# Robinatp/YOLO_Tensorflow

Hardware: AMD Instinct MI355X
Metric: images_per_sec (higher is better)
Workload: dtype bf16; 1 GPU; YOLOv3 416x416 batch=32 per GPU, bf16: conv stack + head decode + threshold + TF-NMS; global_batch=32, input=uint8 NHWC resident in HBM, weights=seeded synthetic darknet stream (seed 0), parallelism=dp1

## Files before the change

### yolo_tensorflow_amd/csrc/conv_block.hip

```cpp
#include "kernels.h"
#include "device_common.h"
#include <type_traits>

constexpr int CB_B = 13;
constexpr int CB_T = CB_B + 2;
constexpr int CB_TPIX = CB_T * CB_T;
constexpr int CB_TSUB = (CB_TPIX + 15) / 16;
constexpr int CB_OPIX = CB_B * CB_B;
constexpr int CB_OSUB = (CB_OPIX + 15) / 16;
constexpr int CB_C = 128, CB_M = 64;
constexpr int CB_NW = 8;
constexpr int CB_NJ = 6;
constexpr int CB_X_BYTES = CB_TSUB * 16 * CB_C * 2;
constexpr int CB_MPITCH = CB_M * 2 + 16;
constexpr int CB_MID_BYTES = CB_TSUB * 16 * CB_MPITCH;
constexpr int CB_W1PITCH = CB_C * 2 + 16;
constexpr int CB_W1_BYTES = CB_M * CB_W1PITCH;
constexpr int CB_OPITCH = CB_C * 2 + 16;
constexpr int CB_OUT_BYTES = CB_OSUB * 16 * CB_OPITCH;
constexpr int CB_B1_BYTES = CB_M * 4, CB_B2_BYTES = CB_C * 4;
constexpr int CB_LDS = CB_X_BYTES + CB_MID_BYTES + CB_W1_BYTES + CB_B1_BYTES + CB_B2_BYTES + CB_OUT_BYTES;

template <bool H16>
__global__ __launch_bounds__(64 * CB_NW) void conv_resblock_c128(const BlockArgs a)
{
#if defined(__HIP_DEVICE_COMPILE__)
    extern __shared__ __attribute__((aligned(16))) char smem[];
    if constexpr (H16) fp16_saturating_mode();
    const int tid = threadIdx.x, lane = tid & 63, wave = __builtin_amdgcn_readfirstlane(tid >> 6);
    const int l15 = lane & 15, lq = lane >> 4;
    const int wc = wave & 3, wp = wave >> 2;
    char *const lx_ = smem, *const lmid_ = lx_ + CB_X_BYTES, *const lw1_ = lmid_ + CB_MID_BYTES, *const lb1_ = lw1_ + CB_W1_BYTES, *const lb2_ = lb1_ + CB_B1_BYTES, *const lout_ = lb2_ + CB_B2_BYTES;
    const float slope1 = act_slope(a.act1), slope2 = act_slope(a.act2);
    const int bx = (a.W + CB_B - 1) / CB_B, by = (a.H + CB_B - 1) / CB_B, per_img = bx * by, nblocks = a.N * per_img;
    const int nt = (nblocks - (int)blockIdx.x + (int)gridDim.x - 1) / (int)gridDim.x;

    for (int g = tid; g < CB_M * 16; g += 64 * CB_NW) {
        const int row = g >> 4, piece = g & 15;
        *(uint4 *)(lw1_ + row * CB_W1PITCH + piece * 16) = *(const uint4 *)((const bf16_t *)a.w1 + (size_t)row * a.Kpad1 + piece * 8);
    }
    bf16x8 fw2[2][18];
#pragma unroll
    for (int ct = 0; ct < 2; ++ct)
#pragma unroll
        for (int ks = 0; ks < 18; ++ks)
            fw2[ct][ks] = *(const bf16x8 *)((const bf16_t *)a.w2 + (size_t)(wc * 32 + ct * 16 + l15) * a.Kpad2 + ks * 32 + lq * 8);
    if (tid < CB_M) *(float *)(lb1_ + tid * 4) = a.b1[tid];
    if (tid < CB_C) *(float *)(lb2_ + tid * 4) = a.b2[tid];

    __amdgpu_buffer_rsrc_t rx = buf_rsrc(a.x);
    __amdgpu_buffer_rsrc_t ro = buf_rsrc(a.out);

    struct Blk { int n, y0, x0; };
    auto blk_of = [&](int j) { const int b = (int)blockIdx.x + j * (int)gridDim.x; Blk q; q.n = b / per_img; const int r = b - q.n * per_img; q.y0 = (r / bx) * CB_B; q.x0 = (r - (r / bx) * bx) * CB_B; return q; };
    auto fetch_x = [&](const Blk &q, lds_char *dst) {
        const int cl = lane >> 4, chunk = lane & 15;
#pragma unroll 1
        for (int id = wave; id < CB_T * 4; id += CB_NW) {
            const int r = id >> 2, c = (id & 3) * 4 + cl;
            const int iy = q.y0 - 1 + r, ix = q.x0 - 1 + c;
            const bool ok = (unsigned)iy < (unsigned)a.H && (unsigned)ix < (unsigned)a.W;
            const unsigned off = ok ? (unsigned)((((q.n * a.H + iy) * a.W + ix) * a.x_stride + ((chunk ^ ((c - r) & 7)) * 8)) * 2) : 0x80000000u;
            if (c < CB_T) __builtin_amdgcn_raw_ptr_buffer_load_lds(rx, (lds_void *)(dst + (r * CB_T + (id & 3) * 4) * 256), 16, off, 0, 0, 0);
        }
    };

    typedef const __attribute__((address_space(3))) bf16x8 *lds_frag_p;
    uint32_t mida[CB_NJ];
#pragma unroll
    for (int j = 0; j < CB_NJ; ++j) {
        int q = (wp * CB_NJ + j) * 16 + l15; if (q >= CB_OPIX) q = CB_OPIX - 1;
        const int oy = (q * 5042) >> 16, ox = q - oy * CB_B;
        mida[j] = (uint32_t)(uintptr_t)(lds_char *)lmid_ + (uint32_t)((oy * CB_T + ox) * CB_MPITCH + lq * 16);
        asm volatile("" : "+v"(mida[j]));
    }

    auto block = [&](int it, const lds_char *__restrict__ lx, lds_char *__restrict__ lx_dma, lds_char *__restrict__ lmid, const lds_char *__restrict__ mid_rd,
                     const lds_char *__restrict__ lw1, const lds_char *__restrict__ lb1, const lds_char *__restrict__ lb2, lds_char *__restrict__ lout) {
        const Blk q = blk_of(it);
        static_assert((CB_OPIX * 16 + 64 * CB_NW - 1) / (64 * CB_NW) == 6, "vmcnt below counts the stores of one thread");
        if (it > 0) __builtin_amdgcn_s_waitcnt(waitcnt_imm(6, 0));
        __builtin_amdgcn_s_barrier();
        {
            const int u = wave;
            f32x4 acc[2][4];
#pragma unroll
            for (int s = 0; s < 2; ++s)
#pragma unroll
                for (int ct = 0; ct < 4; ++ct) acc[s][ct] = f32x4{0.f, 0.f, 0.f, 0.f};
            int p0 = (2 * u) * 16 + l15;
            asm volatile("" : "+v"(p0));
            const int p1 = p0 + 16;
            bf16x8 xf[2][2], wf[2][4];
            auto frags = [&](int kk) {
                xf[kk & 1][0] = *(lds_frag_p)(lx + p0 * 256 + (((kk * 4 + lq) ^ (p0 & 7)) << 4));
                xf[kk & 1][1] = *(lds_frag_p)(lx + p1 * 256 + (((kk * 4 + lq) ^ (p1 & 7)) << 4));
#pragma unroll
                for (int ct = 0; ct < 4; ++ct) wf[kk & 1][ct] = *(lds_frag_p)(lw1 + (ct * 16 + l15) * CB_W1PITCH + (kk * 4 + lq) * 16);
            };
            frags(0);
            __builtin_amdgcn_sched_barrier(0);
#pragma unroll
            for (int kk = 0; kk < 4; ++kk) {
                if (kk + 1 < 4) frags(kk + 1);
#pragma unroll
                for (int ct = 0; ct < 4; ++ct) {
                    acc[0][ct] = mma16<H16>(wf[kk & 1][ct], xf[kk & 1][0], acc[0][ct]);
                    acc[1][ct] = mma16<H16>(wf[kk & 1][ct], xf[kk & 1][1], acc[1][ct]);
                }
                __builtin_amdgcn_sched_barrier(0);
            }
#pragma unroll
            for (int s = 0; s < 2; ++s) {
                const int p = s ? p1 : p0;
                if (2 * u + s >= CB_TSUB) continue;
                const int r = (p * 4370) >> 16, col = p - r * CB_T;
                const bool inside = p < CB_TPIX && (unsigned)(q.y0 - 1 + r) < (unsigned)a.H && (unsigned)(q.x0 - 1 + col) < (unsigned)a.W;
#pragma unroll
                for (int ct = 0; ct < 4; ++ct) {
                    uint2 pk = leaky_pack4<H16>(acc[s][ct], *(const __attribute__((address_space(3))) f32x4 *)(lb1 + (ct * 16 + lq * 4) * 4), slope1);
                    if (!inside) pk = uint2{0u, 0u};
                    *(__attribute__((address_space(3))) uint2 *)(lmid + p * CB_MPITCH + (ct * 16 + lq * 4) * 2) = pk;
                }
            }
        }
        __builtin_amdgcn_s_waitcnt(waitcnt_imm(63, 0));
        __builtin_amdgcn_s_barrier();
        if (it + 1 < nt) fetch_x(blk_of(it + 1), lx_dma);
        f32x4 acc2[2][CB_NJ];
#pragma unroll
        for (int ct = 0; ct < 2; ++ct)
#pragma unroll
            for (int j = 0; j < CB_NJ; ++j) acc2[ct][j] = f32x4{0.f, 0.f, 0.f, 0.f};
        bf16x8 fg[3][2];
        auto koff = [](int ks) { const int t = ks >> 1, h = ks & 1, kh = t / 3, kw = t - kh * 3; return (kh * CB_T + kw) * CB_MPITCH + h * 64; };
#pragma unroll
        for (int j = 0; j < 2; ++j) fg[0][j] = *(lds_frag_p)(mid_rd + mida[j] + koff(0));
        __builtin_amdgcn_sched_barrier(0);
#pragma unroll
        for (int ks = 0; ks < 18; ++ks)
#pragma unroll
            for (int g = 0; g < 3; ++g) {
                const int gn = (g + 1) % 3, ksn = g == 2 ? ks + 1 : ks;
                if (ksn < 18) {
#pragma unroll
                    for (int j = 0; j < 2; ++j) fg[gn][j] = *(lds_frag_p)(mid_rd + mida[gn * 2 + j] + koff(ksn));
                }
#pragma unroll
                for (int j = 0; j < 2; ++j) { acc2[0][g * 2 + j] = mma16<H16>(fw2[0][ks], fg[g][j], acc2[0][g * 2 + j]); acc2[1][g * 2 + j] = mma16<H16>(fw2[1][ks], fg[g][j], acc2[1][g * 2 + j]); }
                __builtin_amdgcn_sched_barrier(0);
            }
        auto stage_out = [&](int ct) {
            const f32x4 bv = *(const __attribute__((address_space(3))) f32x4 *)(lb2 + (wc * 32 + ct * 16 + lq * 4) * 4);
#pragma unroll
            for (int j = 0; j < CB_NJ; ++j)
                if (wp * CB_NJ + j < CB_OSUB)
                    *(__attribute__((address_space(3))) uint2 *)(lout + ((wp * CB_NJ + j) * 16 + l15) * CB_OPITCH + (wc * 32 + ct * 16 + lq * 4) * 2) = leaky_pack4<H16>(acc2[ct][j], bv, slope2);
        };
        stage_out(0);
        constexpr int NPIECE = (CB_OPIX * 16 + 64 * CB_NW - 1) / (64 * CB_NW);
        u32x4_t rsv[NPIECE];
#pragma unroll
        for (int k = 0; k < NPIECE; ++k) {
            int g = tid + k * 64 * CB_NW;
            asm volatile("" : "+v"(g));
            const int px = g >> 4, piece = g & 15;
            const int oy = (px * 5042) >> 16, ox = px - oy * CB_B;
            const unsigned pix = (unsigned)((q.n * a.H + q.y0 + oy) * a.W + q.x0 + ox);
            rsv[k] = __builtin_amdgcn_raw_buffer_load_b128(rx, (px < CB_OPIX && q.y0 + oy < a.H && q.x0 + ox < a.W) ? (pix * a.x_stride + piece * 8) * 2 : 0x80000000u, 0, 0);
        }
        stage_out(1);
        __builtin_amdgcn_s_waitcnt(waitcnt_imm(63, 0));
        __builtin_amdgcn_s_barrier();
#pragma unroll
        for (int k = 0; k < NPIECE; ++k) {
            int g = tid + k * 64 * CB_NW;
            asm volatile("" : "+v"(g));
            const int px = g >> 4, piece = g & 15;
            const int oy = (px * 5042) >> 16, ox = px - oy * CB_B;
            const bool ok = px < CB_OPIX && q.y0 + oy < a.H && q.x0 + ox < a.W;
            const unsigned pix = (unsigned)((q.n * a.H + q.y0 + oy) * a.W + q.x0 + ox);
            const u32x4_t r = rsv[k];
            u32x4_t o = *(const __attribute__((address_space(3))) u32x4_t *)(lout + (px < CB_OPIX ? px : 0) * CB_OPITCH + piece * 16);
#pragma unroll
            for (int e = 0; e < 4; ++e) o[e] = pack16x2<H16>(unpack16_lo<H16>(o[e]) + unpack16_lo<H16>(r[e]), unpack16_hi<H16>(o[e]) + unpack16_hi<H16>(r[e]));
            __builtin_amdgcn_raw_buffer_store_b128(o, ro, ok ? (pix * a.out_stride + piece * 8) * 2 : 0x80000000u, 0, OUT_STORE_AUX);
        }
    };
    if (nt > 0) fetch_x(blk_of(0), (lds_char *)lx_);
    __builtin_amdgcn_s_waitcnt(waitcnt_imm(0, 0));
    for (int it = 0; it < nt; ++it) block(it, (const lds_char *)lx_, (lds_char *)lx_, (lds_char *)lmid_, (const lds_char *)(uintptr_t)0, (const lds_char *)lw1_, (const lds_char *)lb1_, (const lds_char *)lb2_, (lds_char *)lout_);
#endif
}

bool conv_resblock_ok(const BlockArgs &a)
{
    const double px = (double)a.N * a.H * a.W;
    if (px * a.x_stride * 2.0 >= 2147483648.0 || px * a.out_stride * 2.0 >= 2147483648.0) return false;
    const long cover = (long)((a.H + CB_B - 1) / CB_B) * ((a.W + CB_B - 1) / CB_B) * CB_B * CB_B;
    if (a.H <= 0 || a.W <= 0 || cover * 100 > (long)a.H * a.W * 115) return false;
    return (a.dt == DT_BF16 || a.dt == DT_F16) && a.C == CB_C && a.Cmid == CB_M &&
           a.Kpad1 >= CB_C && a.Kpad2 >= 9 * CB_M && (a.x_stride % 8) == 0 && a.x_stride >= CB_C && (a.out_stride % 8) == 0 && a.out_stride >= CB_C;
}

hipError_t launch_conv_resblock(const BlockArgs &a, hipStream_t s)
{
    if (!conv_resblock_ok(a)) return hipErrorInvalidValue;
    const bool h16 = a.dt == DT_F16;
    const void *k = h16 ? (const void *)conv_resblock_c128<true> : (const void *)conv_resblock_c128<false>;
    { hipError_t e = conv_opt_in_lds(k, CB_LDS); if (e != hipSuccess) return e; }
    long blocks = (long)a.N * ((a.H + CB_B - 1) / CB_B) * ((a.W + CB_B - 1) / CB_B);
    if (blocks > 256) blocks = 256;
    if (h16) hipLaunchKernelGGL(conv_resblock_c128<true>, dim3((unsigned)blocks), dim3(64 * CB_NW), CB_LDS, s, a);
    else hipLaunchKernelGGL(conv_resblock_c128<false>, dim3((unsigned)blocks), dim3(64 * CB_NW), CB_LDS, s, a);
    return hipGetLastError();
}
```

Baseline: 12560 img/s.

## Add four-wave half-height resblock form to fit two workgroups per CU

Templates the fused 1x1+3x3 residual block kernel on a wave-group count, adding a four-wave variant that processes a 6x13 output strip. In that variant the mid and output LDS buffers are aliased, behind an extra barrier, so two workgroups fit on one CU. At launch, an occupancy query picks the four-wave form with a grid of twice the CU count whenever two blocks can be resident, and falls back to the eight-wave form otherwise. The aim is latency hiding across workgroups. The cost is more halo rows per output pixel, an extra barrier, and the register pressure that comes with launch_bounds(…,2).

```diff
diff --git a/yolo_tensorflow_amd/csrc/conv_block.hip b/yolo_tensorflow_amd/csrc/conv_block.hip
--- a/yolo_tensorflow_amd/csrc/conv_block.hip
+++ b/yolo_tensorflow_amd/csrc/conv_block.hip
@@ -1,38 +1,54 @@
 #include "kernels.h"
 #include "device_common.h"
 #include <type_traits>
+#include <map>
+#include <mutex>
 
 constexpr int CB_B = 13;
 constexpr int CB_T = CB_B + 2;
-constexpr int CB_TPIX = CB_T * CB_T;
-constexpr int CB_TSUB = (CB_TPIX + 15) / 16;
-constexpr int CB_OPIX = CB_B * CB_B;
-constexpr int CB_OSUB = (CB_OPIX + 15) / 16;
 constexpr int CB_C = 128, CB_M = 64;
-constexpr int CB_NW = 8;
-constexpr int CB_NJ = 6;
-constexpr int CB_X_BYTES = CB_TSUB * 16 * CB_C * 2;
 constexpr int CB_MPITCH = CB_M * 2 + 16;
-constexpr int CB_MID_BYTES = CB_TSUB * 16 * CB_MPITCH;
 constexpr int CB_W1PITCH = CB_C * 2 + 16;
 constexpr int CB_W1_BYTES = CB_M * CB_W1PITCH;
 constexpr int CB_OPITCH = CB_C * 2 + 16;
-constexpr int CB_OUT_BYTES = CB_OSUB * 16 * CB_OPITCH;
 constexpr int CB_B1_BYTES = CB_M * 4, CB_B2_BYTES = CB_C * 4;
-constexpr int CB_LDS = CB_X_BYTES + CB_MID_BYTES + CB_W1_BYTES + CB_B1_BYTES + CB_B2_BYTES + CB_OUT_BYTES;
-
-template <bool H16>
-__global__ __launch_bounds__(64 * CB_NW) void conv_resblock_c128(const BlockArgs a)
+template <int NP> struct CbGeom {
+    static constexpr int BR = NP == 2 ? CB_B : 6;
+    static constexpr int TR = BR + 2;
+    static constexpr int TPIX = TR * CB_T;
+    static constexpr int TSUB = (TPIX + 15) / 16;
+    static constexpr int OPIX = BR * CB_B;
+    static constexpr int OSUB = (OPIX + 15) / 16;
+    static constexpr int NW = 4 * NP;
+    static constexpr int NJ = (OSUB + NP - 1) / NP;
+    static constexpr int NG = (NJ + 1) / 2;
+    static constexpr int NPIECE = (OPIX * 16 + 64 * NW - 1) / (64 * NW);
+    static constexpr int X_BYTES = TSUB * 16 * CB_C * 2;
+    static constexpr int MID_BYTES = TSUB * 16 * CB_MPITCH;
+    static constexpr int OUT_BYTES = OSUB * 16 * CB_OPITCH;
+    static constexpr bool ALIAS = NP == 1;
+    static constexpr int MIDOUT_BYTES = ALIAS ? (MID_BYTES > OUT_BYTES ? MID_BYTES : OUT_BYTES) : MID_BYTES + OUT_BYTES;
+    static constexpr int LDS = X_BYTES + MIDOUT_BYTES + CB_W1_BYTES + CB_B1_BYTES + CB_B2_BYTES;
+    static_assert(2 * NW >= TSUB, "stage 1: wave u takes halo sub-tiles 2u, 2u + 1");
+    static_assert(TPIX <= 240 && OPIX < 176, "the divisions by 15 and 13 below are multiplications");
+};
+static_assert(CbGeom<2>::LDS == 162048 && CbGeom<2>::LDS <= 160 * 1024, "eight-wave form: one workgroup per CU");
+static_assert(CbGeom<1>::LDS == 72704 && 2 * CbGeom<1>::LDS <= 160 * 1024, "four-wave form: two workgroups per CU");
+
+template <bool H16, int NP>
+__global__ __launch_bounds__(64 * CbGeom<NP>::NW, 2) void conv_resblock_c128(const BlockArgs a)
 {
 #if defined(__HIP_DEVICE_COMPILE__)
+    typedef CbGeom<NP> G;
+    constexpr int CB_NW = G::NW, CB_NJ = G::NJ, CB_TSUB = G::TSUB, CB_TPIX = G::TPIX, CB_OPIX = G::OPIX, CB_OSUB = G::OSUB, CB_TR = G::TR, CB_BR = G::BR, NPIECE = G::NPIECE;
     extern __shared__ __attribute__((aligned(16))) char smem[];
     if constexpr (H16) fp16_saturating_mode();
     const int tid = threadIdx.x, lane = tid & 63, wave = __builtin_amdgcn_readfirstlane(tid >> 6);
     const int l15 = lane & 15, lq = lane >> 4;
     const int wc = wave & 3, wp = wave >> 2;
-    char *const lx_ = smem, *const lmid_ = lx_ + CB_X_BYTES, *const lw1_ = lmid_ + CB_MID_BYTES, *const lb1_ = lw1_ + CB_W1_BYTES, *const lb2_ = lb1_ + CB_B1_BYTES, *const lout_ = lb2_ + CB_B2_BYTES;
+    char *const lx_ = smem, *const lmid_ = lx_ + G::X_BYTES, *const lout_ = G::ALIAS ? lmid_ : lmid_ + G::MID_BYTES, *const lw1_ = lmid_ + G::MIDOUT_BYTES, *const lb1_ = lw1_ + CB_W1_BYTES, *const lb2_ = lb1_ + CB_B1_BYTES;
     const float slope1 = act_slope(a.act1), slope2 = act_slope(a.act2);
-    const int bx = (a.W + CB_B - 1) / CB_B, by = (a.H + CB_B - 1) / CB_B, per_img = bx * by, nblocks = a.N * per_img;
+    const int bx = (a.W + CB_B - 1) / CB_B, by = (a.H + CB_BR - 1) / CB_BR, per_img = bx * by, nblocks = a.N * per_img;
     const int nt = (nblocks - (int)blockIdx.x + (int)gridDim.x - 1) / (int)gridDim.x;
 
     for (int g = tid; g < CB_M * 16; g += 64 * CB_NW) {
@@ -52,11 +68,11 @@
     __amdgpu_buffer_rsrc_t ro = buf_rsrc(a.out);
 
     struct Blk { int n, y0, x0; };
-    auto blk_of = [&](int j) { const int b = (int)blockIdx.x + j * (int)gridDim.x; Blk q; q.n = b / per_img; const int r = b - q.n * per_img; q.y0 = (r / bx) * CB_B; q.x0 = (r - (r / bx) * bx) * CB_B; return q; };
+    auto blk_of = [&](int j) { const int b = (int)blockIdx.x + j * (int)gridDim.x; Blk q; q.n = b / per_img; const int r = b - q.n * per_img; q.y0 = (r / bx) * CB_BR; q.x0 = (r - (r / bx) * bx) * CB_B; return q; };
     auto fetch_x = [&](const Blk &q, lds_char *dst) {
         const int cl = lane >> 4, chunk = lane & 15;
 #pragma unroll 1
-        for (int id = wave; id < CB_T * 4; id += CB_NW) {
+        for (int id = wave; id < CB_TR * 4; id += CB_NW) {
             const int r = id >> 2, c = (id & 3) * 4 + cl;
             const int iy = q.y0 - 1 + r, ix = q.x0 - 1 + c;
             const bool ok = (unsigned)iy < (unsigned)a.H && (unsigned)ix < (unsigned)a.W;
@@ -78,8 +94,7 @@
     auto block = [&](int it, const lds_char *__restrict__ lx, lds_char *__restrict__ lx_dma, lds_char *__restrict__ lmid, const lds_char *__restrict__ mid_rd,
                      const lds_char *__restrict__ lw1, const lds_char *__restrict__ lb1, const lds_char *__restrict__ lb2, lds_char *__restrict__ lout) {
         const Blk q = blk_of(it);
-        static_assert((CB_OPIX * 16 + 64 * CB_NW - 1) / (64 * CB_NW) == 6, "vmcnt below counts the stores of one thread");
-        if (it > 0) __builtin_amdgcn_s_waitcnt(waitcnt_imm(6, 0));
+        if (it > 0) __builtin_amdgcn_s_waitcnt(waitcnt_imm(NPIECE, 0));
         __builtin_amdgcn_s_barrier();
         {
             const int u = wave;
@@ -132,22 +147,23 @@
         for (int ct = 0; ct < 2; ++ct)
 #pragma unroll
             for (int j = 0; j < CB_NJ; ++j) acc2[ct][j] = f32x4{0.f, 0.f, 0.f, 0.f};
-        bf16x8 fg[3][2];
+        bf16x8 fg[G::NG][2];
         auto koff = [](int ks) { const int t = ks >> 1, h = ks & 1, kh = t / 3, kw = t - kh * 3; return (kh * CB_T + kw) * CB_MPITCH + h * 64; };
 #pragma unroll
         for (int j = 0; j < 2; ++j) fg[0][j] = *(lds_frag_p)(mid_rd + mida[j] + koff(0));
+        auto in_group = [](int g, int j) { return g * 2 + j < CB_NJ; };
         __builtin_amdgcn_sched_barrier(0);
 #pragma unroll
         for (int ks = 0; ks < 18; ++ks)
 #pragma unroll
-            for (int g = 0; g < 3; ++g) {
-                const int gn = (g + 1) % 3, ksn = g == 2 ? ks + 1 : ks;
+            for (int g = 0; g < G::NG; ++g) {
+                const int gn = (g + 1) % G::NG, ksn = g == G::NG - 1 ? ks + 1 : ks;
                 if (ksn < 18) {
 #pragma unroll
-                    for (int j = 0; j < 2; ++j) fg[gn][j] = *(lds_frag_p)(mid_rd + mida[gn * 2 + j] + koff(ksn));
+                    for (int j = 0; j < 2; ++j) if (in_group(gn, j)) fg[gn][j] = *(lds_frag_p)(mid_rd + mida[gn * 2 + j] + koff(ksn));
                 }
 #pragma unroll
-                for (int j = 0; j < 2; ++j) { acc2[0][g * 2 + j] = mma16<H16>(fw2[0][ks], fg[g][j], acc2[0][g * 2 + j]); acc2[1][g * 2 + j] = mma16<H16>(fw2[1][ks], fg[g][j], acc2[1][g * 2 + j]); }
+                for (int j = 0; j < 2; ++j) if (in_group(g, j)) { acc2[0][g * 2 + j] = mma16<H16>(fw2[0][ks], fg[g][j], acc2[0][g * 2 + j]); acc2[1][g * 2 + j] = mma16<H16>(fw2[1][ks], fg[g][j], acc2[1][g * 2 + j]); }
                 __builtin_amdgcn_sched_barrier(0);
             }
         auto stage_out = [&](int ct) {
@@ -157,8 +173,8 @@
                 if (wp * CB_NJ + j < CB_OSUB)
                     *(__attribute__((address_space(3))) uint2 *)(lout + ((wp * CB_NJ + j) * 16 + l15) * CB_OPITCH + (wc * 32 + ct * 16 + lq * 4) * 2) = leaky_pack4<H16>(acc2[ct][j], bv, slope2);
         };
+        if constexpr (G::ALIAS) __builtin_amdgcn_s_barrier();
         stage_out(0);
-        constexpr int NPIECE = (CB_OPIX * 16 + 64 * CB_NW - 1) / (64 * CB_NW);
         u32x4_t rsv[NPIECE];
 #pragma unroll
         for (int k = 0; k < NPIECE; ++k) {
@@ -203,15 +219,45 @@
            a.Kpad1 >= CB_C && a.Kpad2 >= 9 * CB_M && (a.x_stride % 8) == 0 && a.x_stride >= CB_C && (a.out_stride % 8) == 0 && a.out_stride >= CB_C;
 }
 
+static hipError_t resblock_residency(bool h16, int *per_cu, int *cus)
+{
+    static std::mutex mu;
+    static std::map<std::pair<int, bool>, std::pair<int, int>> known;
+    int dev = 0;
+    hipError_t e = hipGetDevice(&dev); if (e != hipSuccess) return e;
+    std::lock_guard<std::mutex> g(mu);
+    auto it = known.find({dev, h16});
+    if (it == known.end()) {
+        const void *k = h16 ? (const void *)conv_resblock_c128<true, 1> : (const void *)conv_resblock_c128<false, 1>;
+        int n = 0, m = 0;
+        e = conv_opt_in_lds(k, CbGeom<1>::LDS); if (e != hipSuccess) return e;
+        e = h16 ? hipOccupancyMaxActiveBlocksPerMultiprocessor(&n, conv_resblock_c128<true, 1>, 64 * CbGeom<1>::NW, CbGeom<1>::LDS)
+                : hipOccupancyMaxActiveBlocksPerMultiprocessor(&n, conv_resblock_c128<false, 1>, 64 * CbGeom<1>::NW, CbGeom<1>::LDS);
+        if (e != hipSuccess) return e;
+        e = hipDeviceGetAttribute(&m, hipDeviceAttributeMultiprocessorCount, dev); if (e != hipSuccess) return e;
+        it = known.insert({{dev, h16}, {n, m}}).first;
+    }
+    *per_cu = it->second.first; *cus = it->second.second;
+    return hipSuccess;
+}
+
+template <bool H16, int NP>
+static hipError_t launch_resblock_form(const BlockArgs &a, long max_grid, hipStream_t s)
+{
+    typedef CbGeom<NP> G;
+    { hipError_t e = conv_opt_in_lds((const void *)conv_resblock_c128<H16, NP>, G::LDS); if (e != hipSuccess) return e; }
+    long blocks = (long)a.N * ((a.H + G::BR - 1) / G::BR) * ((a.W + CB_B - 1) / CB_B);
+    if (blocks > max_grid) blocks = max_grid;
+    hipLaunchKernelGGL((conv_resblock_c128<H16, NP>), dim3((unsigned)blocks), dim3(64 * G::NW), G::LDS, s, a);
+    return hipGetLastError();
+}
+
 hipError_t launch_conv_resblock(const BlockArgs &a, hipStream_t s)
 {
     if (!conv_resblock_ok(a)) return hipErrorInvalidValue;
     const bool h16 = a.dt == DT_F16;
-    const void *k = h16 ? (const void *)conv_resblock_c128<true> : (const void *)conv_resblock_c128<false>;
-    { hipError_t e = conv_opt_in_lds(k, CB_LDS); if (e != hipSuccess) return e; }
-    long blocks = (long)a.N * ((a.H + CB_B - 1) / CB_B) * ((a.W + CB_B - 1) / CB_B);
-    if (blocks > 256) blocks = 256;
-    if (h16) hipLaunchKernelGGL(conv_resblock_c128<true>, dim3((unsigned)blocks), dim3(64 * CB_NW), CB_LDS, s, a);
-    else hipLaunchKernelGGL(conv_resblock_c128<false>, dim3((unsigned)blocks), dim3(64 * CB_NW), CB_LDS, s, a);
-    return hipGetLastError();
-}
+    int per_cu = 0, cus = 0;
+    { hipError_t e = resblock_residency(h16, &per_cu, &cus); if (e != hipSuccess) return e; }
+    if (per_cu >= 2) return h16 ? launch_resblock_form<true, 1>(a, 2L * cus, s) : launch_resblock_form<false, 1>(a, 2L * cus, s);
+    return h16 ? launch_resblock_form<true, 2>(a, 256, s) : launch_resblock_form<false, 2>(a, 256, s);
+}
```

After: 12620 img/s (median of 6 runs). No clear change (+0.5%).
